# tomasz-pres/face-super-resolution

Hardware: AMD Instinct MI355X
Metric: images/sec (64->256 4x SR) at batch 32/GPU (higher is better)
Workload: dtype fp16; 1 GPU; FaceEnhanceNet full (6x10 RCAB, 64ch) inference 64->256, fp16 (BASELINE configs[1]; its bf16 run is the 'bf16' leg); global_batch=32, per_gpu_batch=32, parallelism=single

## Files before the change

### face-super-resolution_amd/csrc/conv3x3.hip

```cpp
#include "fen_common.h"

#include <type_traits>

extern "C" int fen_maxpool2(int dtype, int B, int H, int W, int C, const void* x, void* y, void* stream);

namespace {

#ifdef FEN_STAMPS
#define FEN_STAMP(i)                                                                          \
    do {                                                                                      \
        __builtin_amdgcn_sched_barrier(0);                                                    \
        unsigned long long _rt, _mt;                                                          \
        asm volatile("s_memrealtime %0\n\ts_memtime %1\n\ts_waitcnt lgkmcnt(0)"                 \
                     : "=s"(_rt), "=s"(_mt)::"memory");                                       \
        __builtin_amdgcn_sched_barrier(0);                                                    \
        if (d.loss_part && (threadIdx.x & 63) == 0 && (i) < 16) {        \
            unsigned long long* _p =                                                          \
                (unsigned long long*)d.loss_part + ((size_t)blockIdx.x * 8 + (threadIdx.x >> 6)) * 32; \
            _p[2 * (i)] = _rt;                                                                \
            _p[2 * (i) + 1] = _mt;                                                            \
        }                                                                                     \
    } while (0)
#else
#define FEN_STAMP(i) \
// ... 1069 lines not shown
    const int wr = wave & 3, wc = wave >> 2;
    const int q = lane >> 4, c16 = lane & 15;
    const int H = d.H, W = d.W, Cin = d.Cin, Cout = d.Cout;
    const int ncot = Cout / V_COT;
    const int bid = xcd_block();
    const int cot = bid % ncot, co0 = cot * V_COT;
    const int nslot = gridDim.x / ncot, slot = bid / ncot;
    const int twn = (W + 15) >> 4, tpi = twn * ((H + 15) >> 4);
    const int ntiles = d.B * tpi;
    const int nmine = slot < ntiles ? (ntiles - slot + nslot - 1) / nslot : 0;
    const int npan = Cin >> 6;
    const int nsteps = nmine * npan * 9;
    if (nsteps == 0) return;
    const i32x4 xr4 = make_rsrc(d.x, (unsigned)((size_t)d.B * H * W * Cin * 2));
    const i32x4 wr4 = make_rsrc(d.w, (unsigned)((size_t)9 * Cout * Cin * 2));

    auto issue_w = [&](int slot_i, int tap, int pn) {
        const unsigned base = lds_addr(wring + slot_i * V_WSLOT) + 4 * wl * 1024;
        const int so = (tap * Cout + co0) * Cin * 2 + pn * 128;
#pragma unroll
        for (int k = 0; k < 4; ++k) {
            const int sl = (4 * wl + k) * 64 + lane;
            const int r = sl >> 3, pc = sl & 7;
#ifndef CVX_NOW
            dma16(wr4, base + k * 1024, so + (r * Cin + (pc ^ ((r >> 1) & 7)) * 8) * 2);
#endif
        }
    };
    auto issue_hk = [&](int par, int t, int pn, int k) {
        const int b = t / tpi, tile = t - b * tpi;
        const int h0 = (tile / twn) << 4, w0 = (tile % twn) << 4;
        const unsigned base = lds_addr(hbuf + par * V_HSLOT) + wl * 1024;
        const int sl = (wl + 4 * k) * 64 + lane;
        const int p = sl >> 3, pc = sl & 7;
        const int hr = p / HALO, hc = p - hr * HALO;
        const int gh = h0 + hr - 1, gw = w0 + hc - 1;
        const bool in = p < HP && (unsigned)gh < (unsigned)H && (unsigned)gw < (unsigned)W;
        const int voff = in ? (((b * H + gh) * W + gw) * Cin + (pc ^ (hc & 7)) * 8) * 2 + pn * 128 : V_BAD;
#ifndef CVX_NOH
        dma16(xr4, __builtin_amdgcn_readfirstlane(base + k * 4096), voff);
#endif
    };
    auto issue_h = [&](int par, int t, int pn) {
#pragma unroll 1
        for (int k = 0; k < 11; ++k) issue_hk(par, t, pn, k);
    };
    const int aoff0 = swz(wc * 64 + c16, q), aoff1 = swz(wc * 64 + c16, 4 + q);
    auto load = [&](int wslot, int par, int kh, int kw, int kk, uint4 (&A)[MT], uint4 (&Bf)[NT]) {
        const char* pa = wring + wslot * V_WSLOT + (kk ? aoff1 : aoff0);
#pragma unroll
        for (int m = 0; m < MT; ++m) A[m] = *(const uint4*)(pa + m * 2048);
        const char* pb = hbuf + par * V_HSLOT + hcol(c16 + kw, kk * 4 + q) + (wr * NT + kh) * (HALO * 128);
#pragma unroll
        for (int n = 0; n < NT; ++n) Bf[n] = *(const uint4*)(pb + n * (HALO * 128));
    };
    f32x4 acc[MT][NT];
    auto mma = [&](const uint4 (&A)[MT], const uint4 (&Bf)[NT]) {
#pragma unroll
        for (int m = 0; m < MT; ++m)
#pragma unroll
            for (int n = 0; n < NT; ++n) mma16<T>(acc[m][n], A[m], Bf[n]);
    };


    if (hwave) {
        issue_h(0, slot, 0);
        asm volatile("s_waitcnt vmcnt(0)" ::: "memory");
    } else {
        for (int s = 0; s < 3 && s < nsteps; ++s) issue_w(s, s, 0);
        if (nsteps > 2) asm volatile("s_waitcnt vmcnt(8)" ::: "memory");
        else if (nsteps > 1) asm volatile("s_waitcnt vmcnt(4)" ::: "memory");
        else asm volatile("s_waitcnt vmcnt(0)" ::: "memory");
    }
    asm volatile("s_waitcnt lgkmcnt(0)" ::: "memory");
    __builtin_amdgcn_s_barrier();
    uint4 A0[MT], B0[NT], A1[MT], B1[NT];
    load(0, 0, 0, 0, 0, A0, B0);
#pragma unroll
    for (int m = 0; m < MT; ++m)
#pragma unroll
        for (int n = 0; n < NT; ++n) acc[m][n] = f32x4{0.f, 0.f, 0.f, 0.f};

    int s = 0, gp = 0;
    for (int j = 0; j < nmine; ++j) {
        for (int pn = 0; pn < npan; ++pn, ++gp) {
            const int par = gp & 1;
            const int pn3 = pn + 1 < npan ? pn + 1 : 0;
#pragma unroll 1
            for (int kh = 0; kh < 3; ++kh) {
#pragma unroll
            for (int kw = 0; kw < 3; ++kw, ++s) {
                const int tap = kh * 3 + kw;
                if (s + 1 < nsteps) {
                    if (!hwave) {
                        if (s + 2 < nsteps) asm volatile("s_waitcnt vmcnt(4)" ::: "memory");
                        else asm volatile("s_waitcnt vmcnt(0)" ::: "memory");
                    } else if (kw == 2 && kh == 2) {
                        asm volatile("s_waitcnt vmcnt(0)" ::: "memory");
                    }
                    asm volatile("s_waitcnt lgkmcnt(0)" ::: "memory");
#ifndef CVX_NOBAR
                    __builtin_amdgcn_s_barrier();
#endif
                    if (hwave) {
#ifndef CVX_HALO_BURST
                        if (kw == 0 && gp + 1 < nmine * npan) {
                            const int tn = pn + 1 < npan ? slot + j * nslot : slot + (j + 1) * nslot;
                            const int pnn = pn + 1 < npan ? pn + 1 : 0;
                            const int k1 = kh < 2 ? 4 * kh + 4 : 11;
#pragma unroll 1
                            for (int k = 4 * kh; k < k1; ++k) issue_hk(par ^ 1, tn, pnn, k);
                        }
#else
                        if (kw == 0 && kh == 0 && gp + 1 < nmine * npan) {
                            if (pn + 1 < npan) issue_h(par ^ 1, slot + j * nslot, pn + 1);
                            else issue_h(par ^ 1, slot + (j + 1) * nslot, 0);
                        }
#endif
                    } else if (s + 3 < nsteps) {
                        issue_w((s + 3) & 3, (tap + 3) % 9, tap + 3 < 9 ? pn : pn3);
                    }
                }
                __builtin_amdgcn_sched_barrier(0);
                load(s & 3, par, kh, kw, 1, A1, B1);
                __builtin_amdgcn_sched_barrier(0);
                mma(A0, B0);
                __builtin_amdgcn_sched_barrier(0);
                if (kw < 2) load((s + 1) & 3, par, kh, kw + 1, 0, A0, B0);
                else if (kh < 2) load((s + 1) & 3, par, kh + 1, 0, 0, A0, B0);
                else if (pn + 1 < npan) load((s + 1) & 3, par ^ 1, 0, 0, 0, A0, B0);
                __builtin_amdgcn_sched_barrier(0);
                mma(A1, B1);
                __builtin_amdgcn_sched_barrier(0);
            }
            }
        }
        const int t = slot + j * nslot;
        const int b = t / tpi, tile = t - b * tpi;
        const int h0 = (tile / twn) << 4, w0 = (tile % twn) << 4;
        const EpiConst<MT> ec = epi_consts<MT>(d, co0 + wc * 64 + q * 4);
#ifndef CVX_NOEPI
        conv_epilogue<T, V_COT, 4, 2, EPIC, true>(d, acc, b, t, h0, w0, co0, nullptr, red, ec);
#else
        if (acc[0][0][0] == 12345.f) conv_epilogue<T, V_COT, 4, 2, EPIC, true>(d, acc, b, t, h0, w0, co0, nullptr, red, ec);
#endif
#pragma unroll
        for (int m = 0; m < MT; ++m)
#pragma unroll
            for (int n = 0; n < NT; ++n) acc[m][n] = f32x4{0.f, 0.f, 0.f, 0.f};
        if (s < nsteps) load(s & 3, gp & 1, 0, 0, 0, A0, B0);
    }
}

int g_num_cus = 0;

int conv_variant() {
    static int v = -1;
    if (v < 0) {
        const char* e = getenv("FEN_CONV_VARIANT");
        v = e ? atoi(e) : 0;
    }
    return v;
}

template <typename T, int COT, int WR, int WC, int EPIC>
int launch_p(const fen_conv_desc* d, hipStream_t s) {
    const int tpi = ((d->W + 15) >> 4) * ((d->H + 15) >> 4);
    const int ntiles = d->B * tpi;
    const int ncot = ((d->Cout + 15) & ~15) / COT;
    if (g_num_cus == 0) {
        int dev = 0;
        (void)hipGetDevice(&dev);
        (void)hipDeviceGetAttribute(&g_num_cus, hipDeviceAttributeMultiprocessorCount, dev);
        if (g_num_cus <= 0) g_num_cus = 256;
    }
    int grid = g_num_cus;
    grid -= grid % ncot;
    const int maxg = ntiles * ncot;
    if (grid > maxg) grid = maxg;
    const size_t lds = 9 * COT * 128 + 2 * HALO_SLOT + WR * COT * 4 + 64;
    static bool attr_set = false;
    if (!attr_set) {
        (void)hipFuncSetAttribute((const void*)k_conv3x3_p<T, COT, WR, WC, EPIC>,
                                  hipFuncAttributeMaxDynamicSharedMemorySize, (int)lds);
        attr_set = true;
    }
    hipLaunchKernelGGL((k_conv3x3_p<T, COT, WR, WC, EPIC>), dim3(grid), dim3(64 * WR * WC), lds, s, *d);
    FEN_CHECK_LAUNCH();
    return FEN_OK;
}

template <typename T, int EPIC>
int launch_g(const fen_conv_desc* d, hipStream_t s) {
    const int tpi = ((d->W + 15) >> 4) * ((d->H + 15) >> 4);
    const int ntiles = d->B * tpi;
    const int ncot = d->Cout / 64;
    if (g_num_cus == 0) {
        int dev = 0;
        (void)hipGetDevice(&dev);
        (void)hipDeviceGetAttribute(&g_num_cus, hipDeviceAttributeMultiprocessorCount, dev);
        if (g_num_cus <= 0) g_num_cus = 256;
    }
    int grid = g_num_cus;
    grid -= grid % ncot;
    const int maxg = ntiles * ncot;
    if (grid > maxg) grid = maxg;
    static bool attr_set = false;
    if (!attr_set) {
        (void)hipFuncSetAttribute((const void*)k_conv3x3_g<T, EPIC>, hipFuncAttributeMaxDynamicSharedMemorySize, G_LDS);
        attr_set = true;
    }
    hipLaunchKernelGGL((k_conv3x3_g<T, EPIC>), dim3(grid), dim3(512), G_LDS, s, *d);
    FEN_CHECK_LAUNCH();
    return FEN_OK;
}

template <typename T, int EPIC>
int launch_v(const fen_conv_desc* d, hipStream_t s) {
    const int tpi = ((d->W + 15) >> 4) * ((d->H + 15) >> 4);
    const int ntiles = d->B * tpi;
    const int ncot = d->Cout / V_COT;
    if (g_num_cus == 0) {
        int dev = 0;
        (void)hipGetDevice(&dev);
        (void)hipDeviceGetAttribute(&g_num_cus, hipDeviceAttributeMultiprocessorCount, dev);
        if (g_num_cus <= 0) g_num_cus = 256;
    }
    int grid = g_num_cus;
    grid -= grid % ncot;
    if (grid < ncot) grid = ncot;
    const int maxg = ntiles * ncot;
    if (grid > maxg) grid = maxg;
    static bool attr_set = false;
    if (!attr_set) {
        (void)hipFuncSetAttribute((const void*)k_conv3x3_v<T, EPIC>, hipFuncAttributeMaxDynamicSharedMemorySize, V_LDS);
        attr_set = true;
    }
    hipLaunchKernelGGL((k_conv3x3_v<T, EPIC>), dim3(grid), dim3(512), V_LDS, s, *d);
    FEN_CHECK_LAUNCH();
    return FEN_OK;
}

bool conv_v_ok(const fen_conv_desc* d) {
    static int on = -1;
    if (on < 0) {
        const char* e = getenv("FEN_CONV_V");
        on = e ? atoi(e) : 1;
    }
    const int items = d->B * ((d->H + 15) >> 4) * ((d->W + 15) >> 4) * (d->Cout / V_COT);
    int ncu = g_num_cus;
    if (ncu == 0) {
        int dev = 0;
        (void)hipGetDevice(&dev);
        (void)hipDeviceGetAttribute(&ncu, hipDeviceAttributeMultiprocessorCount, dev);
        if (ncu <= 0) ncu = 256;
        g_num_cus = ncu;
    }
    return on && conv_variant() != 1 && items >= ncu && d->Cin % 64 == 0 && d->Cin >= 128 && d->Cout % V_COT == 0 &&
           d->s2d_in == 0 && d->s2d_out == 0 && !(d->epi & (FEN_EPI_SHUFFLE | FEN_EPI_UNSHUFFLE | FEN_EPI_LAST)) &&
           (size_t)d->B * d->H * d->W * d->Cin * 2 < (size_t)V_BAD && (size_t)9 * d->Cout * d->Cin * 2 < (size_t)V_BAD;
}

template <typename T, int COT, int EPIC = -1>
int launch_s(const fen_conv_desc* d, hipStream_t s) {
    const int tpi = ((d->W + 15) >> 4) * ((d->H + 15) >> 4);
    const int coutp = (d->Cout + 15) & ~15;
    dim3 grid(d->B * tpi, coutp / COT);
    const size_t lds = HALO_BYTES + 3 * COT * 128;
    static bool attr_set = false;
    if (!attr_set) {
        (void)hipFuncSetAttribute((const void*)k_conv3x3_s<T, COT, EPIC>, hipFuncAttributeMaxDynamicSharedMemorySize,
                                  (int)lds);
        attr_set = true;
    }
    hipLaunchKernelGGL((k_conv3x3_s<T, COT, EPIC>), grid, dim3(256), lds, s, *d);
    FEN_CHECK_LAUNCH();
    return FEN_OK;
}

template <typename T>
int conv_dispatch(const fen_conv_desc* d, hipStream_t s) {
    const int epi = d->epi;
    constexpr bool H16 = sizeof(T) == 2;
    const bool small = (size_t)d->B * d->H * d->W * 128 < (size_t)0x7fff0000;
    const bool s2d = d->s2d_in > 0 || d->s2d_out > 0;
    const bool persist = H16 && d->Cin == 64 && small && !(epi & FEN_EPI_UNSHUFFLE) && conv_variant() != 1 && !s2d;
    if (epi & FEN_EPI_LAST) {
        if (d->Cout > 4 || !d->lr || d->scale <= 0 || d->H % d->scale || d->W % d->scale) return FEN_EINVAL;
        if (epi & ~(FEN_EPI_LAST | FEN_EPI_BIAS)) return FEN_EUNSUPPORTED;
        if (fen_detail::conv_last_fast_ok(d) && conv_variant() != 1) return fen_detail::launch_conv_last(d, s);
        return launch_s<T, 16>(d, s);
    }
    if (!d->y) return FEN_EINVAL;
    if (epi & FEN_EPI_SHUFFLE) {
        if (d->Cout % 64) return FEN_EUNSUPPORTED;
        if (epi & (FEN_EPI_PRELU_BWD | FEN_EPI_POOL | FEN_EPI_DOT) || d->res[0] || d->res[1] || d->res[2])
            return FEN_EUNSUPPORTED;
    }
    if ((epi & FEN_EPI_UNSHUFFLE) && ((d->H | d->W) & 1)) return FEN_EINVAL;
    if (d->y_pool) {
        if constexpr (H16) {
            constexpr int B_ = FEN_EPI_BIAS;
            const bool dense = !d->res[0] && !d->res[1] && !d->res[2];
            if (dense && epi == (B_ | FEN_EPI_PRELU) && d->Cout % 64 == 0 && conv_variant() == 0) {
                if (persist) return launch_g<T, B_ | FEN_EPI_PRELU | EPIC_MPOOL>(d, s);
                if (conv_v_ok(d)) return launch_v<T, B_ | FEN_EPI_PRELU | EPIC_MPOOL>(d, s);
            }
        }
        fen_conv_desc d2 = *d;
        d2.y_pool = nullptr;
        d2.y_images = 0;
        const int rc = conv_dispatch<T>(&d2, s);
        if (rc != FEN_OK) return rc;
        return fen_maxpool2(d->dtype, d->B, d->H, d->W, d->Cout, d->y, d->y_pool, s);
    }
    if (d->Cout % 64 == 0) {
        if constexpr (H16) {
            if (persist) {
                const int nres = d->res[0] ? (d->res[1] ? (d->res[2] ? 3 : 2) : 1) : 0;
                bool dense = true;
                for (int k = nres; k < 3; ++k) dense = dense && !d->res[k];
                const int key = dense && conv_variant() != 2 ? (epi | (nres << 8)) : -1;
                constexpr int B_ = FEN_EPI_BIAS;
                if (conv_variant() == 3 && key == (B_ | FEN_EPI_PRELU)) return launch_p<T, 64, 4, 1, B_ | FEN_EPI_PRELU>(d, s);
                if (conv_variant() != 5 && conv_variant() != 3) {
                    switch (key) {
                        case B_ | FEN_EPI_PRELU: return launch_g<T, B_ | FEN_EPI_PRELU>(d, s);
                        case B_ | FEN_EPI_POOL: return launch_p<T, 64, 4, 2, B_ | FEN_EPI_POOL>(d, s);
                        case B_ | (1 << 8): return launch_g<T, B_ | (1 << 8)>(d, s);
                        case B_ | FEN_EPI_PRELU | FEN_EPI_SHUFFLE: return launch_g<T, B_ | FEN_EPI_PRELU | FEN_EPI_SHUFFLE>(d, s);
                        case FEN_EPI_PRELU_BWD: return launch_p<T, 64, 4, 2, FEN_EPI_PRELU_BWD>(d, s);
                        case FEN_EPI_RELU_BWD: return launch_g<T, FEN_EPI_RELU_BWD>(d, s);
                        case 0: return launch_g<T, 0>(d, s);
                        case 1 << 8: return launch_g<T, 1 << 8>(d, s);
                        case 2 << 8: return launch_g<T, 2 << 8>(d, s);
                        case 3 << 8: return launch_g<T, 3 << 8>(d, s);
                        case FEN_EPI_DOT: return launch_g<T, FEN_EPI_DOT>(d, s);
                        case FEN_EPI_DOT | (1 << 8): return launch_g<T, FEN_EPI_DOT | (1 << 8)>(d, s);
                        default: break;
                    }
                }
                switch (key) {
                    case B_ | FEN_EPI_PRELU: return launch_p<T, 64, 4, 2, B_ | FEN_EPI_PRELU>(d, s);
                    case B_ | FEN_EPI_POOL: return launch_p<T, 64, 4, 2, B_ | FEN_EPI_POOL>(d, s);
                    case B_ | (1 << 8): return launch_p<T, 64, 4, 2, B_ | (1 << 8)>(d, s);
                    case B_ | FEN_EPI_PRELU | FEN_EPI_SHUFFLE:
                        return launch_p<T, 64, 4, 2, B_ | FEN_EPI_PRELU | FEN_EPI_SHUFFLE>(d, s);
                    case FEN_EPI_PRELU_BWD: return launch_p<T, 64, 4, 2, FEN_EPI_PRELU_BWD>(d, s);
                    case 0: return launch_p<T, 64, 4, 2, 0>(d, s);
                    case 1 << 8: return launch_p<T, 64, 4, 2, 1 << 8>(d, s);
                    case 2 << 8: return launch_p<T, 64, 4, 2, 2 << 8>(d, s);
                    case 3 << 8: return launch_p<T, 64, 4, 2, 3 << 8>(d, s);
                    default: return launch_p<T, 64, 4, 2, -1>(d, s);
                }
            }
        }
        if constexpr (H16) {
            if (conv_v_ok(d)) {
                const int nres = d->res[0] ? (d->res[1] ? (d->res[2] ? 3 : 2) : 1) : 0;
                bool dense = true;
                for (int k = nres; k < 3; ++k) dense = dense && !d->res[k];
                constexpr int B_ = FEN_EPI_BIAS;
                switch (dense ? (epi | (nres << 8)) : -1) {
                    case B_ | FEN_EPI_PRELU: return launch_v<T, B_ | FEN_EPI_PRELU>(d, s);
                    case B_: return launch_v<T, B_>(d, s);
                    case FEN_EPI_PRELU_BWD: return launch_v<T, FEN_EPI_PRELU_BWD>(d, s);
                    case FEN_EPI_RELU_BWD: return launch_v<T, FEN_EPI_RELU_BWD>(d, s);
                    case 0: return launch_v<T, 0>(d, s);
                    default: break;
                }
            }
        }
        if constexpr (H16) {
#ifndef CONV_S_GENERIC
            if (!d->res[0] && !d->res[1] && !d->res[2] && !s2d) {
                if (epi == (FEN_EPI_PRELU_BWD | FEN_EPI_UNSHUFFLE))
                    return launch_s<T, 64, FEN_EPI_PRELU_BWD | FEN_EPI_UNSHUFFLE>(d, s);
                if (epi == 0) return launch_s<T, 64, 0>(d, s);
            }
#endif
        }
        return launch_s<T, 64>(d, s);
    }
    if (d->Cout % 16 == 0) return launch_s<T, 16>(d, s);
    return FEN_EUNSUPPORTED;
}

}

extern "C" int fen_conv3x3(const fen_conv_desc* d, void* stream) {
    if (!d || !d->x || !d->w || d->B <= 0 || d->H <= 0 || d->W <= 0 || d->Cin <= 0 || d->Cout <= 0)
        return FEN_EINVAL;
    if (d->dtype != FEN_F32 && d->dtype != FEN_BF16 && d->dtype != FEN_F16) return FEN_EINVAL;
    if ((d->Cin * (d->dtype == FEN_F32 ? 4 : 2)) % 16) return FEN_EUNSUPPORTED;
    const int epi = d->epi;
    if ((epi & FEN_EPI_BIAS) && !d->bias) return FEN_EINVAL;
    if ((epi & (FEN_EPI_PRELU | FEN_EPI_PRELU_BWD)) && !d->alpha) return FEN_EINVAL;
    if ((epi & (FEN_EPI_PRELU_BWD | FEN_EPI_DOT | FEN_EPI_RELU_BWD)) && !d->pre_in) return FEN_EINVAL;
    if (epi & ~0x10ff) return FEN_EINVAL;
    if ((epi & FEN_EPI_RELU_BWD) &&
        (epi & (FEN_EPI_PRELU_BWD | FEN_EPI_DOT | FEN_EPI_LAST | FEN_EPI_SHUFFLE | FEN_EPI_UNSHUFFLE)))
        return FEN_EUNSUPPORTED;
    if ((epi & (FEN_EPI_POOL | FEN_EPI_PRELU_BWD | FEN_EPI_DOT)) && !d->part) return FEN_EINVAL;
    if (d->y_images < 0 || d->y_images > d->B || (d->y_images && !d->y_pool)) return FEN_EINVAL;
    if (d->y_pool && (!(epi & FEN_EPI_PRELU) || ((d->H | d->W) & 1) || d->s2d_in || d->s2d_out ||
                      (epi & (FEN_EPI_SHUFFLE | FEN_EPI_UNSHUFFLE | FEN_EPI_LAST | FEN_EPI_POOL | FEN_EPI_DOT))))
        return FEN_EUNSUPPORTED;
    {
        const int np = !!(epi & FEN_EPI_POOL) + !!(epi & FEN_EPI_PRELU_BWD) + !!(epi & FEN_EPI_DOT);
        if (np > 1) return FEN_EUNSUPPORTED;
    }
    if ((epi & FEN_EPI_DOT) && (epi & (FEN_EPI_UNSHUFFLE | FEN_EPI_LAST))) return FEN_EUNSUPPORTED;
    if (d->s2d_in < 0 || d->s2d_out < 0 || (d->s2d_in && d->s2d_out)) return FEN_EINVAL;
    if (d->s2d_in && (d->s2d_in % 64 || d->Cin != 4 * d->s2d_in)) return FEN_EINVAL;
    if (d->s2d_out && (d->s2d_out % 64 || d->Cout != 4 * d->s2d_out)) return FEN_EINVAL;
    if ((d->s2d_in || d->s2d_out) && (epi & (FEN_EPI_LAST | FEN_EPI_SHUFFLE | FEN_EPI_UNSHUFFLE)))
        return FEN_EUNSUPPORTED;
    if ((epi & (FEN_EPI_SHUFFLE | FEN_EPI_UNSHUFFLE)) == (FEN_EPI_SHUFFLE | FEN_EPI_UNSHUFFLE))
        return FEN_EUNSUPPORTED;
    hipStream_t s = (hipStream_t)stream;
    switch (d->dtype) {
        case FEN_BF16: return conv_dispatch<bf16>(d, s);
        case FEN_F16: return conv_dispatch<f16>(d, s);
        default: return conv_dispatch<float>(d, s);
    }
}
```

### face-super-resolution_amd/src/hip/lib.py

```python
from __future__ import annotations

import ctypes
import os
from ctypes import POINTER, Structure, c_float, c_int, c_size_t, c_void_p

_HERE = os.path.dirname(os.path.abspath(__file__))
LIB_PATH = os.environ.get("FEN_HIP_LIB", os.path.join(_HERE, "libfen_hip.so"))

F32, BF16, F16 = 0, 1, 2

EPI_BIAS = 1
EPI_PRELU = 2
EPI_SHUFFLE = 4
EPI_PRELU_BWD = 8
EPI_UNSHUFFLE = 16
EPI_POOL = 32
EPI_LAST = 64
EPI_DOT = 128
EPI_RELU_BWD = 4096


class AdamwJob(Structure):
    _fields_ = [("p", c_void_p), ("g", c_void_p), ("m", c_void_p), ("v", c_void_p), ("step", c_void_p),
                ("n", c_size_t)]


class ConvDesc(Structure):
    _fields_ = [
        ("dtype", c_int), ("B", c_int), ("H", c_int), ("W", c_int), ("Cin", c_int), ("Cout", c_int),
        ("x", c_void_p), ("w", c_void_p), ("bias", c_void_p), ("epi", c_int), ("alpha", c_void_p),
        ("y", c_void_p), ("y_pre", c_void_p), ("res", c_void_p * 3), ("pre_in", c_void_p),
        ("part", c_void_p), ("lr", c_void_p), ("scale", c_int), ("clamp", c_int), ("hr", c_void_p),
        ("dout", c_void_p), ("l1_scale", c_float), ("loss_part", c_void_p), ("debug", c_int),
        ("s2d_in", c_int), ("s2d_out", c_int),
        ("pre_elide", c_int), ("post_in", c_void_p), ("y_pool", c_void_p), ("y_images", c_int),
    ]


class ColsumJob(Structure):
    _fields_ = [("part", c_void_p), ("out", c_void_p), ("rows", c_int), ("cols", c_int), ("scale", c_float),
                ("accumulate", c_int)]


class PackJob(Structure):
    _fields_ = [("w", c_void_p), ("out", c_void_p), ("mode", c_int), ("Cout", c_int), ("Cin", c_int)]


class RcabDeferredDesc(Structure):
    _fields_ = [
        ("dtype", c_int), ("B", c_int), ("H", c_int), ("W", c_int), ("C", c_int), ("Cr", c_int),
        ("x", c_void_p), ("tp", c_void_p), ("pp", c_void_p), ("pfc1", c_void_p), ("pfc2", c_void_p),
        ("res_scale", c_float), ("inv_hw", c_float), ("ps", c_void_p), ("pmean", c_void_p), ("phid", c_void_p),
        ("xo", c_void_p), ("w1", c_void_p), ("b1", c_void_p), ("alpha", c_void_p), ("w2", c_void_p),
        ("b2", c_void_p), ("t", c_void_p), ("part", c_void_p), ("z1", c_void_p), ("a1", c_void_p),
        ("stamps", c_void_p),
    ]


class RcabBwdDesc(Structure):
    _fields_ = [
        ("dtype", c_int), ("B", c_int), ("H", c_int), ("W", c_int), ("C", c_int),
        ("dt", c_void_p), ("w2t", c_void_p), ("z1", c_void_p), ("alpha", c_void_p), ("w1t", c_void_p),
        ("dy", c_void_p), ("dz1", c_void_p), ("dalpha_part", c_void_p), ("dx", c_void_p),
        ("dot_t", c_void_p), ("dot_part", c_void_p),
        ("se_part", c_void_p), ("se_s", c_void_p), ("se_mean", c_void_p), ("se_hid", c_void_p),
        ("se_w1", c_void_p), ("se_w2", c_void_p), ("se_dw1p", c_void_p), ("se_dw2p", c_void_p),
        ("se_res_scale", c_float), ("se_Cr", c_int), ("dres", c_void_p),
    ]


GS_MAXNB = 20


class GroupStripDesc(Structure):
    _fields_ = [
        ("dtype", c_int), ("B", c_int), ("H", c_int), ("W", c_int), ("C", c_int), ("Cr", c_int), ("nb", c_int),
        ("res_scale", c_float), ("x", c_void_p), ("y", c_void_p),
        ("w1", c_void_p * GS_MAXNB), ("b1", c_void_p * GS_MAXNB), ("alpha", c_void_p * GS_MAXNB),
        ("w2", c_void_p * GS_MAXNB), ("b2", c_void_p * GS_MAXNB), ("fc1", c_void_p * GS_MAXNB),
        ("fc2", c_void_p * GS_MAXNB), ("s_out", c_void_p * GS_MAXNB),
        ("wg", c_void_p), ("bg", c_void_p), ("work", c_void_p), ("work_bytes", c_size_t),
        ("save", c_int), ("sv_x", c_void_p * GS_MAXNB), ("sv_z1", c_void_p * GS_MAXNB),
        ("sv_a1", c_void_p * GS_MAXNB), ("sv_t", c_void_p * GS_MAXNB), ("sv_mean", c_void_p * GS_MAXNB),
        ("sv_hid", c_void_p * GS_MAXNB), ("x_last", c_void_p), ("status", c_void_p), ("fault", c_int),
        ("pre_elide", c_int),
    ]


class GroupStripChainTail(Structure):
    _fields_ = [("w", c_void_p), ("bias", c_void_p), ("skip", c_void_p), ("y", c_void_p)]


class GroupStripBwdDesc(Structure):
    _fields_ = [
        ("dtype", c_int), ("B", c_int), ("H", c_int), ("W", c_int), ("C", c_int), ("Cr", c_int), ("nb", c_int),
        ("res_scale", c_float), ("dy", c_void_p), ("dx", c_void_p), ("dres", c_void_p), ("wgt", c_void_p),
        ("w1t", c_void_p * GS_MAXNB), ("w2t", c_void_p * GS_MAXNB), ("alpha", c_void_p * GS_MAXNB),
        ("fc1", c_void_p * GS_MAXNB), ("fc2", c_void_p * GS_MAXNB), ("z1", c_void_p * GS_MAXNB),
        ("t", c_void_p * GS_MAXNB), ("s", c_void_p * GS_MAXNB), ("mean", c_void_p * GS_MAXNB),
        ("hid", c_void_p * GS_MAXNB), ("dt", c_void_p * GS_MAXNB), ("dz1", c_void_p * GS_MAXNB),
        ("dalpha_part", c_void_p * GS_MAXNB), ("dw1p", c_void_p * GS_MAXNB), ("dw2p", c_void_p * GS_MAXNB),
        ("work", c_void_p), ("work_bytes", c_size_t), ("status", c_void_p), ("fault", c_int),
        ("a1", c_void_p * GS_MAXNB),
    ]


class RcabC128Desc(Structure):
    _fields_ = [
        ("dtype", c_int), ("B", c_int), ("H", c_int), ("W", c_int), ("C", c_int), ("Cr", c_int), ("mode", c_int),
        ("res_scale", c_float), ("x", c_void_p), ("tp", c_void_p), ("pp", c_void_p), ("pfc1", c_void_p),
        ("pfc2", c_void_p), ("ps", c_void_p), ("xo", c_void_p), ("w", c_void_p), ("bias", c_void_p),
        ("alpha", c_void_p), ("res", c_void_p), ("y", c_void_p), ("z1", c_void_p), ("part", c_void_p),
    ]


class WgradDesc(Structure):
    _fields_ = [
        ("dtype", c_int), ("B", c_int), ("H", c_int), ("W", c_int), ("Cin", c_int), ("Cout", c_int),
        ("cout_valid", c_int), ("x", c_void_p), ("dy", c_void_p), ("dw", c_void_p), ("db", c_void_p),
        ("accumulate", c_int), ("work", c_void_p),
    ]


_SIGS = {
    "fen_conv3x3": (c_int, [POINTER(ConvDesc), c_void_p]),
    "fen_wgrad_work_floats": (c_size_t, [POINTER(WgradDesc)]),
    "fen_wgrad3x3": (c_int, [POINTER(WgradDesc), c_void_p]),
    "fen_wgrad_multi_work_floats": (c_size_t, [c_int, c_void_p]),
    "fen_wgrad3x3_multi": (c_int, [c_int, c_void_p, c_void_p]),
    "fen_rcab_deferred_supported": (c_int, [c_int] * 6),
    "fen_rcab_bwd_se_supported": (c_int, [c_int] * 6),
    "fen_rcab_deferred": (c_int, [POINTER(RcabDeferredDesc), c_void_p]),
    "fen_rcab_bwd": (c_int, [POINTER(RcabBwdDesc), c_void_p]),
    "fen_rcab_group_end": (c_int, [POINTER(RcabDeferredDesc)] + [c_void_p] * 5),
    "fen_group_strip_supported": (c_int, [c_int] * 7),
    "fen_group_strip_work_bytes": (c_size_t, [c_int, c_int]),
    "fen_group_strip": (c_int, [POINTER(GroupStripDesc), c_void_p]),
    "fen_group_strip_chain_work_bytes": (c_size_t, [c_int, c_int, c_int]),
    "fen_group_strip_chain_prepare": (c_int, [POINTER(GroupStripDesc), c_int, POINTER(GroupStripChainTail),
                                              c_void_p]),
    "fen_group_strip_chain": (c_int, [POINTER(GroupStripDesc), c_int, POINTER(GroupStripChainTail), c_void_p]),
    "fen_group_strip_bwd_supported": (c_int, [c_int] * 7),
    "fen_group_strip_bwd_work_bytes": (c_size_t, [c_int, c_int]),
    "fen_group_strip_bwd_dal_rows": (c_int, [c_int, c_int]),
    "fen_group_strip_bwd": (c_int, [POINTER(GroupStripBwdDesc), c_void_p]),
    "fen_rcab_c128_supported": (c_int, [c_int] * 6),
    "fen_rcab_c128_tiles": (c_int, [c_int] * 2),
    "fen_rcab_c128": (c_int, [POINTER(RcabC128Desc), c_void_p]),
    "fen_conv_first_fwd": (c_int, [c_int] * 6 + [c_void_p] * 4 + [c_void_p]),
    "fen_conv_first_fwd_ex": (c_int, [c_int] * 6 + [c_void_p] * 5 + [c_float, c_void_p, c_void_p]),
    "fen_conv_first_work_floats": (c_size_t, [c_int] * 5),
    "fen_conv_first_wgrad": (c_int, [c_int] * 6 + [c_void_p] * 4 + [c_int, c_void_p, c_void_p]),
    "fen_conv_last_dgrad_part_rows": (c_size_t, [c_int] * 3),
    "fen_conv_last_bwd_supported": (c_int, [c_int] * 6),
    "fen_conv_last_bwd": (c_int, [c_int] * 6 + [c_void_p] * 9 + [c_void_p]),
    "fen_conv_last_dgrad": (c_int, [c_int] * 6 + [c_void_p] * 7 + [c_void_p]),
    "fen_se_fwd": (c_int, [c_int, c_int, c_int, c_int, c_float] + [c_void_p] * 6 + [c_void_p]),
    "fen_se_fused": (c_int, [c_int] * 6 + [c_float] + [c_void_p] * 7 + [c_float, c_void_p, c_void_p, c_void_p]),
    "fen_se_apply": (c_int, [c_int] * 4 + [c_void_p, c_void_p, c_float, c_void_p, c_void_p, c_void_p]),
    "fen_pool_parts": (c_size_t, [c_int]),
    "fen_pool_dot": (c_int, [c_int] * 4 + [c_void_p] * 3 + [c_void_p]),
    "fen_se_bwd": (c_int, [c_int] * 4 + [c_float, c_float] + [c_void_p] * 9 + [c_void_p]),
    "fen_se_bwd_fused": (c_int, [c_int] * 6 + [c_float, c_float] + [c_void_p] * 11 + [c_void_p]),
    "fen_se_bwd_apply": (c_int, [c_int] * 4 + [c_void_p, c_void_p, c_float, c_void_p, c_void_p, c_void_p]),
    "fen_bicubic_down4": (c_int, [c_int] * 4 + [c_void_p, c_void_p, c_void_p]),
    "fen_colsum": (c_int, [c_int, c_int, c_void_p, c_float, c_void_p, c_int, c_void_p]),
    "fen_colsum_multi": (c_int, [c_int, c_void_p, c_void_p]),
    "fen_pack_conv_w": (c_int, [c_int] * 4 + [c_void_p, c_void_p, c_void_p]),
    "fen_pack_table_bytes": (c_size_t, [c_int]),
    "fen_pack_table": (c_int, [c_int, c_int, c_void_p, c_void_p, POINTER(c_size_t)]),
    "fen_pack_multi": (c_int, [c_int, c_int, c_void_p, c_size_t, c_void_p]),
    "fen_packed_elems": (c_size_t, [c_int] * 3),
    "fen_nchw_to_nhwc": (c_int, [c_int] * 6 + [c_void_p, c_void_p, c_void_p]),
    "fen_prelu_bwd_unshuffle": (c_int, [c_int] * 5 + [c_void_p] * 5 + [c_void_p]),
    "fen_nhwc_to_nchw": (c_int, [c_int] * 5 + [c_void_p, c_void_p, c_void_p]),
    "fen_sumsq_parts": (c_int, [c_size_t]),
    "fen_sumsq": (c_int, [c_size_t, c_void_p, c_void_p, c_void_p]),
    "fen_optim_prepare": (c_int, [c_int, c_void_p, c_float, c_float, c_float, c_float, c_void_p, c_void_p]),
    "fen_adamw": (c_int, [c_size_t] + [c_void_p] * 5 + [c_float, c_float, c_float, c_void_p]),
    "fen_scale": (c_int, [c_size_t, c_void_p, c_float, c_void_p]),
    "fen_maxpool2": (c_int, [c_int] * 5 + [c_void_p] * 3),
    "fen_maxpool2_bwd_relu": (c_int, [c_int] * 5 + [c_void_p] * 4),
    "fen_feat_loss_parts": (c_int, []),
    "fen_feat_loss": (c_int, [c_int, c_size_t, c_void_p, c_int, c_float, c_void_p, c_int, c_void_p, c_void_p]),
    "fen_ssim_parts": (c_size_t, [c_int] * 4),
    "fen_ssim_work_floats": (c_size_t, [c_int] * 4),
    "fen_ssim_ex": (c_int, [c_int] * 5 + [c_void_p] * 3 + [c_int, c_float, c_float, c_void_p, c_void_p, c_float, c_int,
                                                          c_void_p, c_void_p]),
    "fen_ssim": (c_int, [c_int] * 5 + [c_void_p] * 3 + [c_int, c_float, c_float, c_void_p, c_void_p, c_float, c_int,
                                                        c_void_p]),
    "fen_msssim_work_floats": (c_size_t, [c_int] * 5),
    "fen_msssim": (c_int, [c_int] * 5 + [c_void_p] * 3 + [c_int, c_float, c_float, c_void_p, c_int, c_void_p, c_void_p,
                                                          c_void_p, c_float, c_int, c_void_p]),
    "fen_augment_u8": (c_int, [c_int, c_int] + [c_void_p] * 5),
    "fen_bn_work_floats": (c_size_t, [c_int]),
    "fen_bn_stats": (c_int, [c_int, c_size_t, c_int, c_void_p, c_float, c_float] + [c_void_p] * 5),
    "fen_bn_apply": (c_int, [c_int, c_size_t, c_int] + [c_void_p] * 5 + [c_float, c_void_p, c_void_p]),
    "fen_bn_bwd": (c_int, [c_int, c_size_t, c_int] + [c_void_p] * 5 + [c_float] + [c_void_p] * 3 +
                   [c_int, c_void_p, c_void_p]),
    "fen_bn_stats_n": (c_int, [c_int, c_int, c_size_t, c_int, c_void_p, c_float, c_float] + [c_void_p] * 5),
    "fen_bn_apply_n": (c_int, [c_int, c_int, c_size_t, c_int] + [c_void_p] * 3 + [c_int] + [c_void_p] * 2 +
                       [c_float, c_void_p, c_void_p]),
    "fen_bn_bwd_n": (c_int, [c_int, c_int, c_size_t, c_int] + [c_void_p] * 5 + [c_float] + [c_void_p] * 3 +
                     [c_int, c_void_p, c_void_p]),
    "fen_subsample2": (c_int, [c_int] * 5 + [c_void_p] * 3),
    "fen_s2d2": (c_int, [c_int] * 5 + [c_void_p] * 2 + [c_int, c_void_p]),
    "fen_s2d_filter": (c_int, [c_int, c_int, c_void_p, c_void_p, c_int, c_void_p]),
    "fen_zero_insert2": (c_int, [c_int] * 5 + [c_void_p] * 3),
    "fen_adamw_multi": (c_int, [c_int, c_void_p] + [c_float] * 7 + [c_void_p]),
    "fen_l1_loss": (c_int, [c_size_t] + [c_void_p] * 3 + [c_float] + [c_void_p] * 3),
    "fen_gan_loss": (c_int, [c_int, c_int, c_void_p, c_float, c_void_p, c_void_p]),
    "fen_gan_loss_bwd": (c_int, [c_int, c_int, c_void_p, c_float, c_void_p, c_void_p, c_void_p]),
    "fen_dhead_work_floats": (c_size_t, [c_int] * 3),
    "fen_dhead_fwd": (c_int, [c_int] * 3 + [c_void_p] * 5 + [c_float, c_int] + [c_void_p] * 4),
    "fen_dhead_bwd": (c_int, [c_int] * 3 + [c_void_p] * 6 + [c_float, c_int] + [c_void_p] * 7),
    "fen_status_word": (c_int, [POINTER(c_void_p), POINTER(c_void_p)]),
    "fen_status_take": (c_int, [c_void_p]),
    "fen_rccl_unique_id": (c_int, [c_void_p]),
    "fen_rccl_init": (c_int, [POINTER(c_void_p), c_void_p, c_int, c_int, c_int]),
    "fen_rccl_allreduce_bucket": (c_int, [c_void_p, c_void_p, c_size_t, c_void_p]),
    "fen_rccl_check": (c_int, [c_void_p]),
    "fen_rccl_destroy": (c_int, [c_void_p]),
    "fen_last_rccl_error": (ctypes.c_char_p, []),
    "fen_rccl_library": (ctypes.c_char_p, []),
    "fen_status_string": (ctypes.c_char_p, [c_int]),
    "fen_last_hip_error": (ctypes.c_char_p, []),
    "fen_build_info": (ctypes.c_char_p, []),
}

EXPORTED = tuple(_SIGS)

_lib = None


class FenError(RuntimeError):
    pass


def load():
    global _lib
    if _lib is not None:
        return _lib
    if not os.path.exists(LIB_PATH):
        raise FenError(
            f"libfen_hip.so not found at {LIB_PATH}: build it with `make -C face-super-resolution_amd/csrc` "
            "or __graft_entry__.build(); the HIP backend has no fallback")
    lib = ctypes.CDLL(LIB_PATH)
    for name, (res, args) in _SIGS.items():
        f = getattr(lib, name)
        f.restype = res
        f.argtypes = args
    _lib = lib
    return lib


def check(code: int, what: str = "") -> None:
    if code != 0:
        msg = load().fen_status_string(code).decode()
        if code == -3:
            msg += f" [{load().fen_last_hip_error().decode()}]"
        elif code == -4:
            msg += f" [{load().fen_last_rccl_error().decode()}]"
        raise FenError(f"{what}: {msg} (status {code})")


STATUS_GS_FWD, STATUS_GS_BWD, STATUS_GS_TABLE = 1, 2, 4

_status = {}


def strip_status_ptr(device) -> int:
    import torch
    dev = torch.device(device)
    key = dev.index if dev.index is not None else torch.cuda.current_device()
    ent = _status.get(key)
    if ent is None:
        hp, dp = c_void_p(), c_void_p()
        with torch.cuda.device(key):
# ... 29 lines not shown
```

### include/fen.h

```cpp
#ifndef FEN_H
#define FEN_H

#include <stddef.h>
#include <stdint.h>

#ifdef __cplusplus
extern "C" {
#endif

typedef enum {
    FEN_OK = 0,
    FEN_EINVAL = -1,
    FEN_EUNSUPPORTED = -2,
    FEN_EHIP = -3,
    FEN_ERCCL = -4
} fen_status;

typedef enum { FEN_F32 = 0, FEN_BF16 = 1, FEN_F16 = 2 } fen_dtype;

enum {
    FEN_EPI_BIAS = 1,
    FEN_EPI_PRELU = 2,
    FEN_EPI_SHUFFLE = 4,
    FEN_EPI_PRELU_BWD = 8,
    FEN_EPI_UNSHUFFLE = 16,
    FEN_EPI_POOL = 32,
    FEN_EPI_LAST = 64,
    FEN_EPI_DOT = 128,
    FEN_EPI_RELU_BWD = 4096
};

typedef struct {
    int dtype;
    int B, H, W, Cin, Cout;
    const void* x;
    const void* w;
    const float* bias;
    int epi;
    const float* alpha;
    void* y;
    void* y_pre;
    const void* res[3];
    const void* pre_in;
    float* part;
    const float* lr;
    int scale;
    int clamp;
    const float* hr;
    void* dout;
    float l1_scale;
    float* loss_part;
    int debug;
    int s2d_in;
    int s2d_out;
    int pre_elide;
    const void* post_in;
    void* y_pool;
    int y_images;
} fen_conv_desc;

int fen_conv3x3(const fen_conv_desc* d, void* stream);

typedef struct {
    int dtype;
    int B, H, W, Cin, Cout;
    int cout_valid;
    const void* x;
    const void* dy;
    float* dw;
    float* db;
    int accumulate;
    float* work;
} fen_wgrad_desc;

size_t fen_wgrad_work_floats(const fen_wgrad_desc* d);
int fen_wgrad3x3(const fen_wgrad_desc* d, void* stream);

#define FEN_WGRAD_MAXJOBS 32
size_t fen_wgrad_multi_work_floats(int n, const fen_wgrad_desc* descs);
int fen_wgrad3x3_multi(int n, const fen_wgrad_desc* descs, void* stream);

int fen_conv_first_fwd(int dtype, int B, int Ci, int H, int W, int C, const float* x,
                       const float* w, const float* bias, void* y, void* stream);
int fen_conv_first_fwd_ex(int dtype, int B, int Ci, int H, int W, int C, const float* x,
                          const float* w, const float* bias, const float* in_mean, const float* in_istd,
                          float act, void* y, void* stream);
size_t fen_conv_first_work_floats(int B, int Ci, int H, int W, int C);
int fen_conv_first_wgrad(int dtype, int B, int Ci, int H, int W, int C, const float* x,
                         const void* dy, float* dw, float* db, int accumulate, float* work,
                         void* stream);

size_t fen_conv_last_dgrad_part_rows(int B, int H, int W);
int fen_conv_last_dgrad(int dtype, int B, int H, int W, int C, int Co, const void* dout,
                        const float* w, const void* pre, const void* post, const float* alpha,
                        void* du, float* part, void* stream);
int fen_conv_last_bwd_supported(int dtype, int B, int H, int W, int C, int Co);
int fen_conv_last_bwd(int dtype, int B, int H, int W, int C, int Co, const void* dout,
                      const float* w, const void* pre, const void* post, const float* alpha,
                      void* du, float* dal_part, float* dw_part, float* db_part, void* stream);

int fen_se_fwd(int B, int C, int Cr, int nparts, float inv_hw, const float* part,
               const float* w1, const float* w2, float* mean, float* hid, float* s, void* stream);
int fen_se_fused(int dtype, int B, int HW, int C, int Cr, int nparts, float inv_hw, const float* part,
                 const float* w1, const float* w2, float* mean, float* hid, float* s, const void* t,
                 float res_scale, const void* x, void* y, void* stream);
int fen_se_apply(int dtype, int B, int HW, int C, const void* t, const float* s, float res_scale,
                 const void* x, void* y, void* stream);
size_t fen_pool_parts(int HW);
int fen_pool_dot(int dtype, int B, int HW, int C, const void* a, const void* b_, float* part,
                 void* stream);
int fen_se_bwd(int B, int C, int Cr, int nparts, float inv_hw, float res_scale,
               const float* part, const float* mean, const float* hid, const float* s,
               const float* w1, const float* w2, float* g, float* dw1p, float* dw2p, void* stream);
int fen_se_bwd_fused(int dtype, int B, int HW, int C, int Cr, int nparts, float inv_hw, float res_scale,
                     const float* part, const float* mean, const float* hid, const float* s,
                     const float* w1, const float* w2, const void* dy, float* g, float* dw1p, float* dw2p,
                     void* dt, void* stream);
int fen_se_bwd_apply(int dtype, int B, int HW, int C, const void* dy, const float* s,
                     float res_scale, const float* g, void* dt, void* stream);


typedef struct {
    int dtype;
    int B, H, W, C, Cr;
    const void* x;
    const void* tp;
    const float* pp;
    const float* pfc1;
    const float* pfc2;
    float res_scale;
    float inv_hw;
    float* ps;
    float* pmean;
    float* phid;
    void* xo;
    const void* w1;
    const float* b1;
    const float* alpha;
    const void* w2;
    const float* b2;
    void* t;
    float* part;
    void* z1;
    void* a1;
    unsigned long long* stamps;
} fen_rcab_deferred_desc;
int fen_rcab_deferred_supported(int dtype, int B, int H, int W, int C, int Cr);
int fen_rcab_deferred(const fen_rcab_deferred_desc* d, void* stream);

int fen_rcab_group_end(const fen_rcab_deferred_desc* d, const void* w, const float* bias, const void* res,
                       void* out, void* stream);

#define FEN_GS_MAXNB 20
typedef struct {
    int dtype;
    int B, H, W, C, Cr, nb;
    float res_scale;
    const void* x;
    void* y;
    const void* w1[FEN_GS_MAXNB];
    const float* b1[FEN_GS_MAXNB];
    const float* alpha[FEN_GS_MAXNB];
    const void* w2[FEN_GS_MAXNB];
    const float* b2[FEN_GS_MAXNB];
    const float* fc1[FEN_GS_MAXNB];
    const float* fc2[FEN_GS_MAXNB];
    float* s_out[FEN_GS_MAXNB];
    const void* wg;
    const float* bg;
    void* work;
    size_t work_bytes;
    int save;
    void* sv_x[FEN_GS_MAXNB];
    void* sv_z1[FEN_GS_MAXNB];
    void* sv_a1[FEN_GS_MAXNB];
    void* sv_t[FEN_GS_MAXNB];
    float* sv_mean[FEN_GS_MAXNB];
    float* sv_hid[FEN_GS_MAXNB];
    void* x_last;
    int* status;
    int fault;
    int pre_elide;
} fen_group_strip_desc;
#define FEN_STATUS_GS_FWD 1
#define FEN_STATUS_GS_BWD 2
#define FEN_STATUS_GS_TABLE 4
int fen_group_strip_supported(int dtype, int B, int H, int W, int C, int Cr, int nb);
size_t fen_group_strip_work_bytes(int B, int H);
int fen_group_strip(const fen_group_strip_desc* d, void* stream);
typedef struct {
    const void* w;
    const float* bias;
    const void* skip;
    void* y;
} fen_group_strip_chain_tail;
size_t fen_group_strip_chain_work_bytes(int B, int H, int ng);
int fen_group_strip_chain_prepare(const fen_group_strip_desc* d, int ng, const fen_group_strip_chain_tail* tail,
                                  void* stream);
int fen_group_strip_chain(const fen_group_strip_desc* d, int ng, const fen_group_strip_chain_tail* tail, void* stream);

typedef struct {
    int dtype;
    int B, H, W, C, Cr;
    int mode;
    float res_scale;
    const void* x;
    const void* tp;
    const float* pp;
    const float* pfc1;
    const float* pfc2;
    float* ps;
    void* xo;
    const void* w;
    const float* bias;
// ... 196 lines not shown
```

Measured before the change: 21830 images/sec.

## Add dedicated persistent kernel for 64->256 conv with PReLU and pixel-shuffle epilogue

Adds a specialized persistent conv3x3 kernel for the upsampler case (Cin=64, Cout=256, bias+PReLU+shuffle). Half the waves stream the halo tile while the others DMA weight slabs into a 4-deep LDS ring, and each tile is computed in two 128-channel passes with double-buffered register fragments. The epilogue writes shuffled output directly using permlane16 swaps. It is routed ahead of the generic kernel by default, and adds a route-query export. It trades generality and high LDS use for better weight/halo reuse on this layer.

```diff
diff --git a/face-super-resolution_amd/csrc/conv3x3.hip b/face-super-resolution_amd/csrc/conv3x3.hip
--- a/face-super-resolution_amd/csrc/conv3x3.hip
+++ b/face-super-resolution_amd/csrc/conv3x3.hip
@@ -1245,6 +1245,200 @@
     }
 }
 
+constexpr int U_WSLAB = 3 * 128 * 64;
+constexpr int U_LDS = 4 * U_WSLAB + HALO_SLOT + (256 + 64) * 4;
+
+template <typename T>
+__global__ __launch_bounds__(512, 1) void k_conv3x3_u(const fen_conv_desc d) {
+    constexpr int MT = 4, NT = 4, NB = NT + 2;
+    extern __shared__ __attribute__((aligned(16))) char smem[];
+    char* wring = smem;
+    char* halo = smem + 4 * U_WSLAB;
+    float* cst = (float*)(halo + HALO_SLOT);
+    const int tid = threadIdx.x, lane = tid & 63, wave = tid >> 6;
+    const int wv = wave_id();
+    const bool hwave = wv < 4;
+    const int wl = wv & 3;
+    const int wr = wave & 3, wc = wave >> 2;
+    const int q = lane >> 4, c16 = lane & 15;
+    const int H = d.H, W = d.W;
+    constexpr int Cout = 256, Cq = 64;
+    const int slot = xcd_block(), nslot = gridDim.x;
+    const int twn = (W + 15) >> 4, tpi = twn * ((H + 15) >> 4);
+    const int ntiles = d.B * tpi;
+    const int nmine = slot < ntiles ? (ntiles - slot + nslot - 1) / nslot : 0;
+    if (nmine == 0) return;
+    const i32x4 xr4 = make_rsrc(d.x, (unsigned)((size_t)d.B * H * W * 128));
+    const i32x4 wr4 = make_rsrc(d.w, (unsigned)(9 * Cout * 128));
+
+    FEN_STAMP(0);
+    auto issue_w = [&](int rs, int pass, int g) {
+        const unsigned base = lds_addr(wring + rs * U_WSLAB) + 6 * wl * 1024;
+        const int kw = g >> 1, kk = g & 1;
+        const int so = (kw * Cout + pass * 128) * 128 + kk * 64;
+#pragma unroll
+        for (int k = 0; k < 6; ++k) {
+            const int sl = (6 * wl + k) * 64 + lane;
+            const int rr = sl >> 2, pc = sl & 3;
+            const int kh = rr >> 7, col = rr & 127;
+            dma16(wr4, base + k * 1024, so + (kh * 3 * Cout + col) * 128 + ((pc ^ ((rr >> 2) & 3)) << 4));
+        }
+    };
+    auto issue_h = [&](int t) {
+        const int b = t / tpi, tile = t - b * tpi;
+        const int h0 = (tile / twn) << 4, w0 = (tile % twn) << 4;
+        const unsigned base = lds_addr(halo);
+#pragma unroll 1
+        for (int k = 0; k < 11; ++k) {
+            const int i = wl + 4 * k;
+            if (i >= HALO_DMA) break;
+            const int sl = i * 64 + lane;
+            const int p = sl >> 3, pc = sl & 7;
+            const int hr = p / HALO, hc = p - hr * HALO;
+            const int gh = h0 + hr - 1, gw = w0 + hc - 1;
+            const bool in = p < HP && (unsigned)gh < (unsigned)H && (unsigned)gw < (unsigned)W;
+            const int voff = in ? (((b * H + gh) * W + gw) * 64 + (pc ^ (hc & 7)) * 8) * 2 : 0x7ffffff0;
+            dma16(xr4, __builtin_amdgcn_readfirstlane(base + i * 1024), voff);
+        }
+    };
+    const int aoff = (wc * 64 + c16) * 64 + ((q ^ ((c16 >> 2) & 3)) << 4);
+    auto loadA = [&](int rs, int kh, uint4 (&A)[MT]) {
+        const char* pa = wring + rs * U_WSLAB + kh * (128 * 64) + aoff;
+#pragma unroll
+        for (int m = 0; m < MT; ++m) A[m] = *(const uint4*)(pa + m * 1024);
+    };
+    auto loadB = [&](int g, uint4 (&Bf)[NB]) {
+        const char* pb = halo + hcol(c16 + (g >> 1), (g & 1) * 4 + q) + (wr * NT) * (HALO * 128);
+#pragma unroll
+        for (int n = 0; n < NB; ++n) Bf[n] = *(const uint4*)(pb + n * (HALO * 128));
+    };
+    f32x4 acc[MT][NT];
+    auto mma = [&](const uint4 (&A)[MT], const uint4 (&Bf)[NB], int kh) {
+#pragma unroll
+        for (int m = 0; m < MT; ++m)
+#pragma unroll
+            for (int n = 0; n < NT; ++n) mma16<T>(acc[m][n], A[m], Bf[n + kh]);
+    };
+
+    if (tid < 256) {
+        cst[tid] = (d.epi & FEN_EPI_BIAS) ? d.bias[4 * (tid % Cq) + tid / Cq] : 0.f;
+        if (tid < 64) cst[256 + tid] = d.alpha[tid];
+    }
+    if (hwave) {
+        issue_h(slot);
+        asm volatile("s_waitcnt vmcnt(0)" ::: "memory");
+    } else {
+        issue_w(0, 0, 0);
+        issue_w(1, 0, 1);
+        issue_w(2, 0, 2);
+        asm volatile("s_waitcnt vmcnt(12)" ::: "memory");
+    }
+    asm volatile("s_waitcnt lgkmcnt(0)" ::: "memory");
+    __builtin_amdgcn_s_barrier();
+    FEN_STAMP(1);
+
+    const int nsteps = nmine * 12;
+    uint4 A0[MT], A1[MT], B0[NB], B1[NB];
+    loadA(0, 0, A0);
+    bool drained = true;
+    int s = 0;
+    for (int j = 0; j < nmine; ++j) {
+        const int t = slot + j * nslot;
+#pragma unroll
+        for (int pass = 0; pass < 2; ++pass) {
+#pragma unroll
+            for (int m = 0; m < MT; ++m)
+#pragma unroll
+                for (int n = 0; n < NT; ++n) acc[m][n] = f32x4{0.f, 0.f, 0.f, 0.f};
+#pragma unroll
+            for (int g = 0; g < 6; ++g, ++s) {
+                const int rs = (2 * pass + g) & 3;
+                if (s + 1 < nsteps) {
+                    if (!hwave) {
+                        if (s + 2 >= nsteps) asm volatile("s_waitcnt vmcnt(0)" ::: "memory");
+                        else if (g < 2 && !drained) asm volatile("s_waitcnt vmcnt(14)" ::: "memory");
+                        else asm volatile("s_waitcnt vmcnt(6)" ::: "memory");
+                    } else if (g == 0 && pass == 0) {
+                        if (!drained) asm volatile("s_waitcnt vmcnt(8)" ::: "memory");
+                        else asm volatile("s_waitcnt vmcnt(0)" ::: "memory");
+                    }
+                    asm volatile("s_waitcnt lgkmcnt(0)" ::: "memory");
+                    __builtin_amdgcn_s_barrier();
+                    if (hwave) {
+                        if (pass == 1 && g == 5 && j + 1 < nmine) issue_h(t + nslot);
+                    } else if (s + 3 < nsteps) {
+                        if (g < 3) issue_w((rs + 3) & 3, pass, g + 3);
+                        else issue_w((rs + 3) & 3, pass ^ 1, g - 3);
+                    }
+                }
+                if (g == 0 && pass == 0) loadB(0, B0);
+                __builtin_amdgcn_sched_barrier(0);
+#pragma unroll
+                for (int kh = 0; kh < 3; ++kh) {
+                    const int st = g * 3 + kh;
+                    if (kh < 2) {
+                        if (st & 1) loadA(rs, kh + 1, A0); else loadA(rs, kh + 1, A1);
+                    } else if (g < 5) {
+                        if (st & 1) loadA((rs + 1) & 3, 0, A0); else loadA((rs + 1) & 3, 0, A1);
+                    }
+                    if (kh == 0 && g < 5) {
+                        if (g & 1) loadB(g + 1, B0); else loadB(g + 1, B1);
+                    }
+                    __builtin_amdgcn_sched_barrier(0);
+                    if (st & 1) {
+                        if (g & 1) mma(A1, B1, kh); else mma(A1, B0, kh);
+                    } else {
+                        if (g & 1) mma(A0, B1, kh); else mma(A0, B0, kh);
+                    }
+                    __builtin_amdgcn_sched_barrier(0);
+                }
+            }
+            FEN_STAMP(2 + 4 * j + 2 * pass);
+            const int b = t / tpi, tile = t - b * tpi;
+            const int h0 = (tile / twn) << 4, w0 = (tile % twn) << 4;
+            const bool full = h0 + 16 <= H && w0 + 16 <= W;
+            const bool okw = w0 + c16 < W;
+#pragma unroll
+            for (int mp = 0; mp < 2; ++mp) {
+                const int c0 = 32 * mp + 16 * (q & 1) + 8 * (q >> 1);
+#pragma unroll
+                for (int n = 0; n < NT; ++n) {
+                    unsigned lo[2], hi[2];
+#pragma unroll
+                    for (int e = 0; e < 2; ++e) {
+                        const int m = 2 * mp + e;
+                        const float4 bb = *(const float4*)(cst + pass * 128 + wc * 64 + m * 16 + 4 * q);
+                        const float4 aa = *(const float4*)(cst + 256 + m * 16 + 4 * q);
+                        const float bias4[4] = {bb.x, bb.y, bb.z, bb.w};
+                        const float al4[4] = {aa.x, aa.y, aa.z, aa.w};
+                        float o[4];
+#pragma unroll
+                        for (int r = 0; r < 4; ++r) {
+                            const float v = acc[m][n][r] + bias4[r];
+                            o[r] = prelu_f(v, al4[r]);
+                        }
+                        lo[e] = pack2<T>(o[0], o[1]);
+                        hi[e] = pack2<T>(o[2], o[3]);
+                    }
+                    const auto s0 = __builtin_amdgcn_permlane16_swap(lo[0], lo[1], false, false);
+                    const auto s1 = __builtin_amdgcn_permlane16_swap(hi[0], hi[1], false, false);
+                    const int h = h0 + wr * NT + n, w = w0 + c16;
+                    if (full || (h < H && okw)) {
+                        const size_t off = ((size_t)(b * 2 * H + 2 * h + pass) * (2 * W) + 2 * w + wc) * Cq + c0;
+                        *(uint4*)((char*)d.y + off * 2) = make_uint4(s0[0], s1[0], s0[1], s1[1]);
+                    }
+                }
+            }
+            drained = !full;
+            FEN_STAMP(3 + 4 * j + 2 * pass);
+            if (s < nsteps) {
+                if (pass == 0) loadB(0, B0);
+                loadA(pass == 0 ? 2 : 0, 0, A0);
+            }
+        }
+    }
+}
+
 int g_num_cus = 0;
 
 int conv_variant() {
@@ -1304,6 +1498,40 @@
         attr_set = true;
     }
     hipLaunchKernelGGL((k_conv3x3_g<T, EPIC>), dim3(grid), dim3(512), G_LDS, s, *d);
+    FEN_CHECK_LAUNCH();
+    return FEN_OK;
+}
+
+int conv_u_grid_cap() {
+    const char* e = getenv("FEN_CONV_U_GRID");
+    return e ? atoi(e) : 0;
+}
+
+bool conv_u_ok(const fen_conv_desc* d) {
+    return conv_variant() == 0 && (d->dtype == FEN_BF16 || d->dtype == FEN_F16) && d->Cin == 64 && d->Cout == 256 &&
+           !d->y_pre && !d->res[0] && !d->res[1] && !d->res[2] && !d->y_pool && !d->s2d_in && !d->s2d_out &&
+           d->epi == (FEN_EPI_BIAS | FEN_EPI_PRELU | FEN_EPI_SHUFFLE) &&
+           (size_t)d->B * d->H * d->W * 128 < (size_t)0x7fff0000;
+}
+
+template <typename T>
+int launch_u(const fen_conv_desc* d, hipStream_t s) {
+    const int ntiles = d->B * ((d->W + 15) >> 4) * ((d->H + 15) >> 4);
+    if (g_num_cus == 0) {
+        int dev = 0;
+        (void)hipGetDevice(&dev);
+        (void)hipDeviceGetAttribute(&g_num_cus, hipDeviceAttributeMultiprocessorCount, dev);
+        if (g_num_cus <= 0) g_num_cus = 256;
+    }
+    const int cap = conv_u_grid_cap();
+    int grid = g_num_cus < ntiles ? g_num_cus : ntiles;
+    if (cap > 0 && cap < g_num_cus) grid = cap;
+    static bool attr_set = false;
+    if (!attr_set) {
+        (void)hipFuncSetAttribute((const void*)k_conv3x3_u<T>, hipFuncAttributeMaxDynamicSharedMemorySize, U_LDS);
+        attr_set = true;
+    }
+    hipLaunchKernelGGL((k_conv3x3_u<T>), dim3(grid), dim3(512), U_LDS, s, *d);
     FEN_CHECK_LAUNCH();
     return FEN_OK;
 }
@@ -1415,6 +1643,7 @@
                 for (int k = nres; k < 3; ++k) dense = dense && !d->res[k];
                 const int key = dense && conv_variant() != 2 ? (epi | (nres << 8)) : -1;
                 constexpr int B_ = FEN_EPI_BIAS;
+                if (conv_u_ok(d)) return launch_u<T>(d, s);
                 if (conv_variant() == 3 && key == (B_ | FEN_EPI_PRELU)) return launch_p<T, 64, 4, 1, B_ | FEN_EPI_PRELU>(d, s);
                 if (conv_variant() != 5 && conv_variant() != 3) {
                     switch (key) {
@@ -1479,6 +1708,11 @@
     return FEN_EUNSUPPORTED;
 }
 
+}
+
+extern "C" int fen_conv3x3_route(const fen_conv_desc* d) {
+    if (!d || !d->x || !d->w || !d->y || !d->bias || !d->alpha || d->B <= 0 || d->H <= 0 || d->W <= 0) return 0;
+    return conv_u_ok(d) ? 1 : 0;
 }
 
 extern "C" int fen_conv3x3(const fen_conv_desc* d, void* stream) {
diff --git a/face-super-resolution_amd/src/hip/lib.py b/face-super-resolution_amd/src/hip/lib.py
--- a/face-super-resolution_amd/src/hip/lib.py
+++ b/face-super-resolution_amd/src/hip/lib.py
@@ -124,6 +124,7 @@
 
 _SIGS = {
     "fen_conv3x3": (c_int, [POINTER(ConvDesc), c_void_p]),
+    "fen_conv3x3_route": (c_int, [POINTER(ConvDesc)]),
     "fen_wgrad_work_floats": (c_size_t, [POINTER(WgradDesc)]),
     "fen_wgrad3x3": (c_int, [POINTER(WgradDesc), c_void_p]),
     "fen_wgrad_multi_work_floats": (c_size_t, [c_int, c_void_p]),
diff --git a/include/fen.h b/include/fen.h
--- a/include/fen.h
+++ b/include/fen.h
@@ -60,6 +60,7 @@
 } fen_conv_desc;
 
 int fen_conv3x3(const fen_conv_desc* d, void* stream);
+int fen_conv3x3_route(const fen_conv_desc* d);
 
 typedef struct {
     int dtype;
```

New measurement: 21910 images/sec (median of 3 runs). Within noise of the previous version (+0.4%).
